# mburger-stsci/nexoclom

Measured on AMD Instinct MI355X. Metric: particle*steps/s, higher is better.
Workload: dtype f64

## Files before the change

### nexoclom_amd/build.py

```python
import os
import shutil
import subprocess
import sys

HERE = os.path.dirname(os.path.abspath(__file__))
SRC = os.path.join(HERE, 'csrc', 'nxc_api.hip')
DEPS = [os.path.join(HERE, 'csrc', f) for f in
        ('nxc_api.hip', 'nxc_kernels.hpp', 'nxc_device.hpp', 'nxc_math.hpp', 'nxc_log_table.hpp',
         'nxc_desc_check.hpp', 'nxc_source_limits.hpp')]
DEPS.append(os.path.join(os.path.dirname(HERE), 'include', 'nexoclom_hip.h'))
OUT = os.path.join(HERE, 'lib', 'libnexoclom_hip.so')
OUT_TWO_ROUNDINGS = os.path.join(HERE, 'lib', 'libnexoclom_hip_2r.so')

FLAGS = ['-O3', '--offload-arch=gfx950', '-ffp-contract=off', '-fno-fast-math',
         '-munsafe-fp-atomics', '-mllvm', '-disable-machine-licm', '-fPIC', '-shared',
         '-std=c++17', '-Wall', '-Wno-unused-function']
if os.environ.get('NXC_EXPERIMENT_KNOBS'):
    FLAGS.append('-DNXC_EXPERIMENT_KNOBS')
FLAGS += os.environ.get('NXC_EXTRA_FLAGS', '').split()


def hipcc():
    exe = shutil.which('hipcc') or '/opt/rocm/bin/hipcc'
    if not os.path.exists(exe):
        raise RuntimeError('hipcc not found; the HIP library cannot be built')
    return exe


def up_to_date(out=OUT):
    if not os.path.exists(out):
        return False
    t = os.path.getmtime(out)
# ... 32 lines not shown
```

### nexoclom_amd/csrc/nxc_api.hip

```cpp
#include <hip/hip_runtime.h>
#include <dlfcn.h>
#include <rccl/rccl.h>

#include <algorithm>
#include <atomic>
#include <cmath>
#include <cstddef>
#include <cstdio>
#include <cstdlib>
#include <cstring>
#include <ctime>
#include <limits>
#include <mutex>
#include <new>
#include <string>
#include <vector>

#include "../../include/nexoclom_hip.h"
#include "nxc_desc_check.hpp"
#include "nxc_kernels.hpp"
#include "nxc_log_table.hpp"

namespace {

// ... 70 lines not shown
    if (!g_rccl.lib) return fail(NXC_ERR_RCCL, std::string("dlopen(librccl): ") + dlerror());
#define SYM(field, name)                                                                     \
    g_rccl.field = reinterpret_cast<decltype(g_rccl.field)>(dlsym(g_rccl.lib, name));        \
    if (!g_rccl.field) return fail(NXC_ERR_RCCL, std::string("dlsym ") + name + " failed");
    SYM(GetUniqueId, "ncclGetUniqueId")
    SYM(CommInitRank, "ncclCommInitRank")
    SYM(AllReduce, "ncclAllReduce")
    SYM(CommDestroy, "ncclCommDestroy")
    SYM(CommAbort, "ncclCommAbort")
    SYM(CommGetAsyncError, "ncclCommGetAsyncError")
    SYM(GetErrorString, "ncclGetErrorString")
#undef SYM
    g_rccl.ok = true;
    return NXC_OK;
}

#define NCCLCHK(expr)                                                                        \
    do {                                                                                     \
        ncclResult_t r_ = (expr);                                                            \
        if (r_ != ncclSuccess)                                                               \
            return fail(NXC_ERR_RCCL, std::string(#expr) + ": " + g_rccl.GetErrorString(r_)); \
    } while (0)

struct PackedLut {
    LutDesc desc{};
    std::vector<unsigned char> bytes;
};
struct LosLutCache {
    int64_t n = 0;
    std::vector<double> v, g;
    PackedLut lut;
};

int lut_cell_host(double x, double xbase, double inv_w, int ncell)
{
    const double s = (x - xbase) * inv_w;
    long long c;
    if (!(s >= 0.0)) c = 0;
    else if (s >= 2147483647.0) c = 2147483647ll;
    else c = (long long)s;
    return (int)std::min<long long>(c, ncell + 1);
}

unsigned long long ordered_key(double v)
{
    unsigned long long b;
    std::memcpy(&b, &v, sizeof b);
    return (b >> 63) ? ~b : (b | 0x8000000000000000ull);
}
double from_ordered_key(unsigned long long k)
{
    const unsigned long long b = (k >> 63) ? (k & 0x7fffffffffffffffull) : ~k;
    double v;
    std::memcpy(&v, &b, sizeof v);
    return v;
}

int pack_lut(const double *xp, const double *fp, int64_t n, PackedLut &out, const char *what,
             int cells_per_node = 4)
{
    if (n < 2 || n > 65000 || !xp || !fp)
        return fail(NXC_ERR_ARG, std::string(what) + ": table needs 2..65000 points");
    for (int64_t j = 0; j + 1 < n; j++)
        if (!(xp[j + 1] > xp[j]))
            return fail(NXC_ERR_ARG, std::string(what) + ": abscissae must be strictly ascending");
    for (int64_t j = 0; j < n; j++)
        if (!std::isfinite(xp[j]) || !std::isfinite(fp[j]))
            return fail(NXC_ERR_ARG, std::string(what) + ": table values must be finite");
    int ncell = 64;
    while (ncell < cells_per_node * n && ncell < 16384) ncell <<= 1;
    const int64_t rows = n + 2;
    const size_t cell_bytes = ((size_t)(ncell + 2) * sizeof(unsigned short) + 31) & ~size_t(31);
    out.bytes.assign((size_t)rows * 32 + cell_bytes, 0);
    double *rec = reinterpret_cast<double *>(out.bytes.data());
    double *fs = rec + 2 * rows;
    rec[0] = -std::numeric_limits<double>::max(); rec[1] = xp[0];
    fs[0] = fp[0]; fs[1] = 0.0;
    for (int64_t j = 0; j < n; j++) {
        const bool last = j + 1 == n;
        rec[2 * (j + 1)] = xp[j];
        rec[2 * (j + 1) + 1] = last ? HUGE_VAL : xp[j + 1];
        fs[2 * (j + 1)] = fp[j];
        fs[2 * (j + 1) + 1] = last ? 0.0 : (fp[j + 1] - fp[j]) / (xp[j + 1] - xp[j]);
        if (!std::isfinite(fs[2 * (j + 1) + 1]))
            return fail(NXC_ERR_ARG, std::string(what) + ": table slopes must be finite");
    }
    rec[2 * (n + 1)] = HUGE_VAL; rec[2 * (n + 1) + 1] = HUGE_VAL;
    fs[2 * (n + 1)] = fp[n - 1]; fs[2 * (n + 1) + 1] = 0.0;
    const double x0 = xp[0], xl = xp[n - 1];
    const double inv_w = (double)ncell / (xl - x0);
    const double xbase = x0 - (xl - x0) / (double)ncell;
    if (!std::isfinite(inv_w) || !std::isfinite(xbase) || !(xbase < x0))
        return fail(NXC_ERR_ARG, std::string(what) + ": abscissa range cannot be indexed");
    unsigned short *cell = reinterpret_cast<unsigned short *>(rec + 4 * rows);
    cell[0] = 0;
    const unsigned long long k_lo = ordered_key(-std::numeric_limits<double>::max());
    const unsigned long long k_hi = ordered_key(std::numeric_limits<double>::max());
    for (int c = 1; c <= ncell + 1; c++) {
        if (lut_cell_host(from_ordered_key(k_hi), xbase, inv_w, ncell) < c)
            return fail(NXC_ERR_ARG, std::string(what) + ": cell index is not onto");
        unsigned long long lo = k_lo, hi = k_hi;
        while (hi - lo > 1) {
            const unsigned long long mid = lo + (hi - lo) / 2;
            if (lut_cell_host(from_ordered_key(mid), xbase, inv_w, ncell) >= c) hi = mid;
            else lo = mid;
        }
        const double first = from_ordered_key(hi);
        const int64_t j = std::upper_bound(xp, xp + n, first) - xp;
        cell[c] = (unsigned short)j;
    }
    out.desc.rec = 0;
    out.desc.fs = 16 * (int)rows;
    out.desc.cell = 32 * (int)rows;
    out.desc.top = ncell + 1;
    out.desc.last = (int)n + 1;
    out.desc.xbase = xbase;
    out.desc.inv_w = inv_w;
    return NXC_OK;
}

LutDesc placed_lut(LutDesc d, size_t base)
{
    d.rec += (int)base; d.fs += (int)base; d.cell += (int)base;
    return d;
}

double sqrt_threshold(double e)
{
    if (!(e > 0) || !std::isfinite(e)) return e;
    double x = e * e;
    if (!std::isfinite(x)) return HUGE_VAL;
    while (std::sqrt(x) > e) x = std::nextafter(x, 0.0);
    while (std::sqrt(std::nextafter(x, HUGE_VAL)) <= e) x = std::nextafter(x, HUGE_VAL);
    return x;
}

StepW make_stepw(double h)
{
    StepW w{};
    w.h = h;
    for (int n = 0; n < 6; n++)
        for (int i = 0; i <= n; i++) w.w[n * (n + 1) / 2 + i] = h * Tableau::A[n + 1][i];
    return w;
}

}

// ... 28 lines not shown
    const void *col0 = nullptr;
    int64_t stride = 0;
    template <typename T> const T *col(int c) const { return static_cast<const T *>(cols[c]); }
    template <typename I> const I *idx() const { return static_cast<const I *>(index); }
};

struct nxc_handle {
    int device = 0;
    int n_cu = 0;
    hipStream_t stream = nullptr;
    hipStream_t copy_stream = nullptr;
    hipStream_t stream2 = nullptr;
    unsigned long long *d_piece_hist = nullptr;
    hipEvent_t ev_piece[33] = {};
    hipEvent_t ev0 = nullptr, ev1 = nullptr;
    bool timed = false;
    char name[256] = {0};

    bool have_forces = false, have_image = false;
    ForceK F{};
    ImageK G{};
    PackedLut force_lut;
    std::vector<double> force_v, force_a;
    int force_cells_per_node = 16;
    int force_lut_cells = 0;
    std::vector<unsigned char> image_part;
    LdsHeader header{};
    LutDesc line_local[NXC_MAX_LINES]{};
    size_t line_start[NXC_MAX_LINES]{};
    int64_t xedges_local = 0, zedges_local = 0;
    unsigned char *d_blob = nullptr;
    size_t blob_cap = 0, force_bytes = 0, all_bytes = 0;
    unsigned char *d_blob_img = nullptr;
    size_t blob_img_cap = 0, img_bytes = 0;

    double *d_image = nullptr;
    size_t npix = 0;
    double *d_packets = nullptr;
    size_t packets_cap = 0;
    int64_t n_packets = 0;
    unsigned *d_order = nullptr;
    double *d_queue = nullptr;
    size_t queue_cap = 0;
    size_t order_cap = 0;
    bool have_order = false;
    int order_key = 0;
    int64_t first_id = 0;
    bool have_bounce = false;
// ... 250 lines not shown

std::mutex g_handles_lock;
std::vector<nxc_handle *> g_handles;

void flush_all_pools()
{
    std::lock_guard<std::mutex> g(g_handles_lock);
    for (nxc_handle *h : g_handles) pool_flush(h);
}

size_t pool_bytes(nxc_handle *h)
{
    std::lock_guard<std::mutex> g(h->pool.lock);
    return h->pool.bytes;
}

int upload_blob(nxc_handle *h)
{
    const size_t hb = NXC_HEADER_BYTES;
    const size_t ib = h->have_image ? h->image_part.size() : 0;
    const size_t limit = 160 * 1024 - 32 - (size_t)(BLOCK_PERSIST / 64) * NXC_WAVE_LDS_BYTES;
    const size_t limit_rows = 160 * 1024 - 32 - (size_t)(BLOCK_PERSIST / 64) * NXC_WAVE_LDS_BYTES_ROWS;
    size_t fb = h->have_forces ? h->force_lut.bytes.size() : 0;
    while (h->have_forces && (hb + fb + ib > limit || hb + fb > limit_rows) &&
           h->force_cells_per_node > 2) {
        h->force_cells_per_node /= 2;
        PackedLut lut;
        int rc2 = pack_lut(h->force_v.data(), h->force_a.data(), (int64_t)h->force_v.size(), lut,
                           "nxc_forces radiation table", h->force_cells_per_node);
        if (rc2) return rc2;
        h->force_lut = std::move(lut);
        h->force_lut_cells = h->force_cells_per_node;
        fb = h->force_lut.bytes.size();
    }
    h->force_bytes = hb + fb;
    h->all_bytes = hb + fb + ib;
    if (h->all_bytes > limit || h->force_bytes > limit_rows)
        return fail(NXC_ERR_ARG, "lookup tables exceed the 160 KiB LDS of a gfx950 CU");
    int rc = ensure(reinterpret_cast<void **>(&h->d_blob), &h->blob_cap, h->all_bytes);
    if (rc) return rc;
    h->F.tab = placed_lut(h->force_lut.desc, hb);
    if (h->have_image) {
        for (int l = 0; l < h->G.n_lines; l++) {
            h->G.line[l] = placed_lut(h->line_local[l], hb + fb + h->line_start[l]);
        }
        h->G.xedges_off = h->xedges_local + (int64_t)(hb + fb);
        h->G.zedges_off = h->zedges_local + (int64_t)(hb + fb);
    }
    h->header.G = h->G;
    HIPCHK(hipMemcpyAsync(h->d_blob, &h->header, sizeof(LdsHeader), hipMemcpyHostToDevice,
                          h->stream));
    if (fb) HIPCHK(hipMemcpyAsync(h->d_blob + hb, h->force_lut.bytes.data(), fb,
                                  hipMemcpyHostToDevice, h->stream));
    if (ib) HIPCHK(hipMemcpyAsync(h->d_blob + hb + fb, h->image_part.data(), ib,
                                  hipMemcpyHostToDevice, h->stream));
    HIPCHK(stream_sync(h));
    if (h->have_image) {
        LdsHeader hdr = h->header;
        for (int l = 0; l < h->G.n_lines; l++)
            hdr.G.line[l] = placed_lut(h->line_local[l], hb + h->line_start[l]);
        hdr.G.xedges_off = h->xedges_local + (int64_t)hb;
// ... 428 lines not shown
int los_tables(nxc_handle *h, const nxc_los_desc *d, LosK &K, std::vector<unsigned char> &blob)
{
    blob.assign((size_t)NXC_HEADER_BYTES, 0);
    std::memcpy(blob.data(), &h->header, sizeof(LdsHeader));
    K.sin_dphi = d->sin_dphi;
    K.sin_2dphi = d->sin_2dphi;
    K.cos_thr = d->cos_threshold;
    K.cos_thr2_lo = d->cos_threshold * d->cos_threshold * (1.0 - 1e-9);
    K.vrplanet = d->vrplanet;
    K.unit_cm2 = d->unit_cm * d->unit_cm;
    K.t0 = d->ladder[0];
    K.log1p_s_inv = 1.0 / std::log1p(d->sin_dphi);
    K.n_lines = d->n_lines;
    K.n_ladder = (int)d->n_ladder;
    K.tan_dphi = std::tan(d->dphi);
    for (int l = 0; l < d->n_lines; l++) {
        const size_t nb = (size_t)d->line_n[l] * sizeof(double);
        LosLutCache &c = h->los_lut[l];
        const bool same = c.n == d->line_n[l] && d->line_n[l] > 0 && c.v.size() * sizeof(double) == nb &&
                          std::memcmp(c.v.data(), d->line_v[l], nb) == 0 &&
                          std::memcmp(c.g.data(), d->line_g[l], nb) == 0;
        if (!same) {
            c.n = 0;
            int rc = pack_lut(d->line_v[l], d->line_g[l], d->line_n[l], c.lut, "g-value table");
            if (rc) return rc;
            c.v.assign(d->line_v[l], d->line_v[l] + d->line_n[l]);
            c.g.assign(d->line_g[l], d->line_g[l] + d->line_n[l]);
            c.n = d->line_n[l];
        }
        K.line[l] = placed_lut(c.lut.desc, blob.size());
        blob.insert(blob.end(), c.lut.bytes.begin(), c.lut.bytes.end());
    }
    return NXC_OK;
}

template <typename T, typename I>
int los_run(nxc_handle *h, const nxc_los_desc *d, int64_t S, const double *sc, int64_t P,
            const T *dx, const T *dy, const T *dz, const T *dvy, const T *dfrac, const I *d_index,
            int64_t index_shift, int64_t n_index, double *radiance, int64_t *npackets, uint8_t *included,
            int64_t used_cap, int64_t *used_pairs, int64_t *n_used)
{
    std::vector<unsigned char> blob;
    LosK K{};
    int rc = los_tables(h, d, K, blob);
    if (rc) return rc;
    K.index_shift = index_shift;
    K.cull = (d->dphi > 0 && d->dphi < 1.5 && std::isfinite(K.tan_dphi)) ? 1 : 0;
// ... 773 lines not shown
                          (unsigned long long)c.unfinished);
            return fail(NXC_ERR_INCOMPLETE, buf);
        }
    }
    return NXC_OK;
}

int nxc_set_forces(nxc_handle *h, const nxc_forces *f)
{
    return guarded([&]() -> int {
    if (!h || !f) return fail(NXC_ERR_ARG, "null argument");
    HIPCHK(hipSetDevice(h->device));
    PackedLut lut;
    const double zero_one[2] = {0.0, 1.0}, zeros[2] = {0.0, 0.0};
    int rc;
    const double *nv = f->radpres ? f->v_tab : zero_one, *na = f->radpres ? f->a_tab : zeros;
    const size_t nn = f->radpres ? (size_t)(f->n_tab > 0 ? f->n_tab : 0) : 2;
    if (f->radpres && (f->n_tab < 2 || !f->v_tab || !f->a_tab)) return fail(NXC_ERR_ARG, "radiation table missing");
    const bool same_table = h->have_forces && h->force_v.size() == nn && !h->force_lut.bytes.empty() &&
                            std::memcmp(h->force_v.data(), nv, nn * sizeof(double)) == 0 &&
                            std::memcmp(h->force_a.data(), na, nn * sizeof(double)) == 0;
    h->force_v.assign(nv, nv + nn);
    h->force_a.assign(na, na + nn);
    h->force_cells_per_node = 8;
#ifdef NXC_EXPERIMENT_KNOBS
    if (const char *e = std::getenv("NXC_FORCE_CELLS")) h->force_cells_per_node = std::max(2, std::atoi(e));
#endif
    if (!same_table || h->force_lut_cells != h->force_cells_per_node) {
        rc = pack_lut(h->force_v.data(), h->force_a.data(), (int64_t)h->force_v.size(), lut,
                      "nxc_forces radiation table", h->force_cells_per_node);
        if (rc) { h->have_forces = false; return rc; }
        h->force_lut = std::move(lut);
        h->force_lut_cells = h->force_cells_per_node;
    }
    h->F.GM = f->GM;
    h->F.vrplanet = f->vrplanet;
    h->F.photo = f->photo;
    h->F.inv_lifetime = f->lifetime > 0 ? 1.0 / f->lifetime : 0.0;
    h->F.grav = f->gravity ? 1 : 0;
    h->F.rad = f->radpres ? 1 : 0;
    h->F.loss = f->lifetime > 0 ? LOSS_LIFETIME : (f->has_photo ? LOSS_PHOTO : LOSS_NONE);
    h->have_forces = true;
    return upload_blob(h);
    });
}

int nxc_set_image(nxc_handle *h, const nxc_image_desc *d)
{
    return guarded([&]() -> int {
    if (!h || !d) return fail(NXC_ERR_ARG, "null argument");
    HIPCHK(hipSetDevice(h->device));
    if (d->nx < 1 || d->nz < 1 || d->nx > 32768 || d->nz > 32768 || !d->xedges || !d->zedges)
        return fail(NXC_ERR_ARG, "image dims/edges invalid");
    if (d->quantity != 0 && d->quantity != 1) return fail(NXC_ERR_ARG, "quantity must be 0 or 1");
    const int nl = d->quantity == 1 ? d->n_lines : 0;
    if (nl < 0 || nl > NXC_MAX_LINES) return fail(NXC_ERR_ARG, "n_lines out of range");
// ... 1 lines not shown
    if (!std::isfinite(d->vrplanet)) return fail(NXC_ERR_ARG, "vrplanet must be finite");
    for (int64_t k = 0; k < d->nx; k++)
        if (!(d->xedges[k + 1] > d->xedges[k])) return fail(NXC_ERR_ARG, "xedges not ascending");
    for (int64_t k = 0; k < d->nz; k++)
        if (!(d->zedges[k + 1] > d->zedges[k])) return fail(NXC_ERR_ARG, "zedges not ascending");

    std::vector<unsigned char> part;
    ImageK G{};
    std::memcpy(G.M, d->M, sizeof G.M);
    G.vrplanet = d->vrplanet;
    G.apix_cm2 = d->apix_cm2;
    G.quantity = d->quantity;
    G.n_lines = nl;
    G.downcast_f32 = d->downcast_f32 ? 1 : 0;
#ifdef NXC_EXPERIMENT_KNOBS
    if (const char *dbg = std::getenv("NXC_DEBUG_IMAGE")) G.dbg = std::atoi(dbg);
#endif
    G.nx = (int)d->nx;
    G.nz = (int)d->nz;
    G.x_is_x = (d->M[0] == 1.0 && d->M[1] == 0.0 && d->M[2] == 0.0 && d->M[3] == 0.0 &&
                d->M[6] == 0.0) ? 1 : 0;
    for (int l = 0; l < nl; l++) {
        PackedLut lut;
        int rc = pack_lut(d->line_v[l], d->line_g[l], d->line_n[l], lut, "g-value table");
        if (rc) return rc;
        h->line_local[l] = lut.desc;
        h->line_start[l] = part.size();
        part.insert(part.end(), lut.bytes.begin(), lut.bytes.end());
    }
    h->xedges_local = (int64_t)part.size();
    const unsigned char *xe = reinterpret_cast<const unsigned char *>(d->xedges);
    part.insert(part.end(), xe, xe + (d->nx + 1) * sizeof(double));
    h->zedges_local = (int64_t)part.size();
    const unsigned char *ze = reinterpret_cast<const unsigned char *>(d->zedges);
    part.insert(part.end(), ze, ze + (d->nz + 1) * sizeof(double));
    G.x_lo = d->xedges[0];
    G.x_inv_step = (double)d->nx / (d->xedges[d->nx] - d->xedges[0]);
    G.z_lo = d->zedges[0];
    G.z_inv_step = (double)d->nz / (d->zedges[d->nz] - d->zedges[0]);
    h->image_part = std::move(part);
    h->G = G;
    h->have_image = true;

    const size_t npix = (size_t)d->nx * (size_t)d->nz;
    if (npix != h->npix) {
        if (h->d_image) HIPCHK(hipFree(h->d_image));
        h->d_image = nullptr; h->npix = 0;
// ... 1643 lines not shown
    const std::vector<u128> maps = pcg_tables(((u128)inc[0] << 64) | inc[1], n);
    const size_t map_bytes = maps.size() * sizeof(u128), out_bytes = (size_t)nvec * count * 8;
    int rc = scratch_for(h, map_bytes + out_bytes);
    if (rc) return rc;
    unsigned char *base = reinterpret_cast<unsigned char *>(h->d_scratch);
    HIPCHK(hipMemcpyAsync(base, maps.data(), map_bytes, hipMemcpyHostToDevice, h->stream));
    PcgK P{};
    P.state = ((u128)state[0] << 64) | state[1];
    P.row0 = row0;
    P.maps = reinterpret_cast<const nxc_u128 *>(base);
    hipLaunchKernelGGL(k_pcg_uniforms, dim3(flat_grid(h, count, NXC_BLOCK)), dim3(NXC_BLOCK), 0,
                       h->stream, P, (int)nvec, count, reinterpret_cast<double *>(base + map_bytes));
    HIPCHK(hipGetLastError());
    HIPCHK(hipMemcpyAsync(out, base + map_bytes, out_bytes, hipMemcpyDeviceToHost, h->stream));
    HIPCHK(stream_sync(h));
    return NXC_OK;
    });
}

int nxc_math_batch(nxc_handle *h, int which, int64_t n, const double *in, const double *in2,
                   double *out)
{
    return guarded([&]() -> int {
    if (!h || n < 0 || (n && (!in || !out)) || which < 0 || which > 4 || (which == 4 && !in2))
        return fail(NXC_ERR_ARG, "bad arguments");
    HIPCHK(hipSetDevice(h->device));
    if (n == 0) return NXC_OK;
    const size_t col = (size_t)n * sizeof(double);
    int rc = scratch_for(h, 3 * col);
    if (rc) return rc;
    double *d = h->d_scratch;
    HIPCHK(hipMemcpyAsync(d, in, col, hipMemcpyHostToDevice, h->stream));
    if (in2) HIPCHK(hipMemcpyAsync(d + n, in2, col, hipMemcpyHostToDevice, h->stream));
    if (!h->d_blob && (rc = upload_blob(h))) return rc;
    hipLaunchKernelGGL(k_math, dim3(flat_grid(h, n, 256)), dim3(256), NXC_HEADER_BYTES, h->stream,
                       h->d_blob, which, n, d, d + n, d + 2 * n);
    HIPCHK(hipGetLastError());
    HIPCHK(hipMemcpyAsync(out, d + 2 * n, col, hipMemcpyDeviceToHost, h->stream));
    HIPCHK(stream_sync(h));
    return NXC_OK;
    });
}

}
```

### nexoclom_amd/csrc/nxc_device.hpp

```cpp
#pragma once
#include <hip/hip_runtime.h>
#include <stdint.h>
#include "nxc_math.hpp"

struct LutDesc {
    int rec, fs, cell;
    int top;
    int last;
    int pad_;
    double xbase;
    double inv_w;
};
typedef LutDesc LutView;

extern __shared__ __align__(32) unsigned char nxc_lds[];

#define NXC_LDS_AS __attribute__((address_space(3)))
#define NXC_GLOBAL_AS __attribute__((address_space(1)))
typedef double nxc_v2d __attribute__((ext_vector_type(2)));

NXC_DEV double lds_f64(int byte_off)
{
    return *(const NXC_LDS_AS double *)(unsigned)byte_off;
}
NXC_DEV int lds_u16(int byte_off)
{
    return *(const NXC_LDS_AS unsigned short *)(unsigned)byte_off;
}

NXC_DEV double2 lds_f64x2(int byte_off)
{
    const nxc_v2d v = *(const NXC_LDS_AS nxc_v2d *)(unsigned)byte_off;
    return make_double2(v.x, v.y);
}

NXC_DEV const LutView &lut_view(const LutDesc &d) { return d; }

NXC_DEV int lut_cell(const LutView &t, double x)
{
    const double s = (x - t.xbase) * t.inv_w;
    unsigned c;
    asm("v_cvt_u32_f64 %0, %1" : "=v"(c) : "v"(s));
    const unsigned top = (unsigned)t.top;
    return (int)(c > top ? top : c);
}

struct LutProbe {
    double x;
    int r;
    double2 a0, a1, b0, b1;
};

NXC_DEV void lut_probe_cell(const LutView &t, double x, LutProbe &p)
{
    p.x = x;
    p.r = lds_u16(t.cell + 2 * lut_cell(t, x));
}

NXC_DEV void lut_probe_rows(const LutView &t, LutProbe &p)
{
    const int ra = t.rec + 16 * p.r, rb = t.fs + 16 * p.r;
    p.a0 = lds_f64x2(ra); p.a1 = lds_f64x2(ra + 16);
    p.b0 = lds_f64x2(rb); p.b1 = lds_f64x2(rb + 16);
}

NXC_DEV LutProbe lut_probe(const LutView &t, double x)
{
    LutProbe p;
    lut_probe_cell(t, x, p);
    lut_probe_rows(t, p);
    return p;
}

NXC_DEV double lut_finish(const LutView &t, const LutProbe &p)
{
    const double x = p.x;
    const bool in0 = x < p.a0.y, in1 = x < p.a1.y;
    double xp = in0 ? p.a0.x : p.a1.x;
    double fp = in0 ? p.b0.x : p.b1.x;
    double sl = in0 ? p.b0.y : p.b1.y;
    if (__builtin_expect(!(in0 || in1), 0)) {
        int r = p.r + 1;
        while (r < t.last && x >= lds_f64(t.rec + 16 * r + 8)) ++r;
        const double2 aw = lds_f64x2(t.rec + 16 * r), bw = lds_f64x2(t.fs + 16 * r);
        xp = aw.x; fp = bw.x; sl = bw.y;
    }
    return sl * (x - xp) + fp;
}

NXC_DEV double lut_interp(const LutView &t, double x) { return lut_finish(t, lut_probe(t, x)); }

enum : int { LOSS_NONE = 0, LOSS_LIFETIME = 1, LOSS_PHOTO = 2 };

struct ForceK {
    double GM, vrplanet, photo, inv_lifetime;
    int grav, rad, loss, pad_;
    LutDesc tab;
};

NXC_DEV bool sunlit(double x, double y, double z)
{
    double s = x * x + z * z;
    return (s > 0x1.0000000000001p+0) || (y < 0.0);
}

template <bool FULL>
NXC_DEV void state_eval(const ForceK &F, const LutView &T, double x, double y, double z, double vy,
                        double &ax, double &ay, double &az, double &ion)
{
    const bool lit = sunlit(x, y, z);
// ... 633 lines not shown
NXC_DEV bool image_weight(const ImageK &G, const ImageRegs &R, double radvel, double fw,
                          double &w_out)
{
    double w = fw;
    if (R.quantity != 0) {
        double gg = 0.0;
        if (R.n_lines == 2) {
            const LutView v0 = lut_view(G.line[0]), v1 = lut_view(G.line[1]);
            LutProbe p0, p1;
            lut_probe_cell(v0, radvel, p0); lut_probe_cell(v1, radvel, p1);
            lut_probe_rows(v0, p0); lut_probe_rows(v1, p1);
            const double g0 = lut_finish(v0, p0);
            gg = g0 + lut_finish(v1, p1);
        } else {
            gg = R.n_lines > 0 ? lut_interp(lut_view(G.line[0]), radvel) : 0.0;
#pragma unroll
            for (int l = 1; l < 4; l++)
                if (l < R.n_lines) gg += lut_interp(lut_view(G.line[l]), radvel);
        }
        w = nxc_div_const(fw * gg, 1e6, lds_header().Wt.rs_1e6);
    }
    w = nxc_div_const(w, G.apix_cm2, lds_header().Wt.rs_apix);
    w_out = w;
    return (__builtin_fabs(w) <= 1.7976931348623157e308) && radvel == radvel;
}

NXC_DEV void image_sample(const ImageK &G, const ImageRegs &R, bool has, double x, double y,
                          double z, double vy, double frac, double *__restrict__ acc2,
                          unsigned long long &binned, unsigned long long &nonfinite)
{
    int pix = -1;
    double radvel = 0.0, fw = 0.0, w = 0.0;
    if (has) pix = image_locate(G, R, x, y, z, vy, frac, radvel, fw, nonfinite);
    bool ok = pix >= 0;
    if (ok && !image_weight(G, R, radvel, fw, w)) { nonfinite++; ok = false; }
    binned += ok;
    image_add_pairs(ok, pix, w, acc2);
}

constexpr int NXC_IMGQ_SLOTS = 128;
constexpr int NXC_IMGQ_BYTES = NXC_IMGQ_SLOTS * (8 + 8 + 4);

struct ImageQueue {
    int head = 0, tail = 0;

    NXC_DEV void push(bool has, int pix, double radvel, double fw, int qoff)
    {
// ... 63 lines not shown
```

### nexoclom_amd/csrc/nxc_kernels.hpp

```cpp
#pragma once
#include "nxc_device.hpp"
#include "nxc_source_limits.hpp"

struct DevCounters {
    unsigned long long particle_steps, samples, samples_binned, nonfinite, bad_step, neg_frac,
        unfinished, queue_head;
    unsigned long long wave_trips;
#ifdef NXC_STAMPS
    unsigned long long stamp[8];
#endif
};

#ifdef NXC_STAMPS
NXC_DEV unsigned long long nxc_stamp()
{
    unsigned long long t;
    __builtin_amdgcn_sched_barrier(0);
    asm volatile("s_memtime %0\n\ts_waitcnt lgkmcnt(0)" : "=s"(t) : : "memory");
    __builtin_amdgcn_sched_barrier(0);
    return t;
}
#define NXC_STAMP(k) do { const unsigned long long t_ = nxc_stamp(); seg[k] += t_ - t_prev; t_prev = t_; } while (0)
#else
#define NXC_STAMP(k) do { } while (0)
// ... 1072 lines not shown
#pragma unroll
    for (int j = 0; j < 8; j++) sink += a[j];
    const unsigned long long t1 = __builtin_amdgcn_s_memtime(), r1 = __builtin_amdgcn_s_memrealtime();
    if ((threadIdx.x & 63) == 0) {
        const size_t w = ((size_t)blockIdx.x * blockDim.x + threadIdx.x) >> 6;
        out[3 * w] = t1 - t0;
        out[3 * w + 1] = r1 - r0;
        out[3 * w + 2] = (unsigned long long)__double_as_longlong(sink);
    }
}

__global__ void __launch_bounds__(64)
k_stall(unsigned long long ticks, unsigned long long *__restrict__ out)
{
    const unsigned long long t0 = __builtin_amdgcn_s_memrealtime();
    unsigned long long now = t0;
    while (now - t0 < ticks) {
        __builtin_amdgcn_s_sleep(127);
        now = __builtin_amdgcn_s_memrealtime();
    }
    if (threadIdx.x == 0 && out) *out = now - t0;
}

__global__ void k_math(const unsigned char *__restrict__ blob, int which, int64_t n,
                       const double *__restrict__ in, const double *__restrict__ in2,
                       double *__restrict__ out)
{
    stage_tables(blob, NXC_HEADER_BYTES);
    for (int64_t i = (int64_t)blockIdx.x * blockDim.x + threadIdx.x; i < n;
         i += (int64_t)gridDim.x * blockDim.x) {
        const double v = in[i];
        double r;
        switch (which) {
        case 0: r = nxc_exp(v); break;
        case 1: r = nxc_log(v); break;
        case 2: r = nxc_cube(v); break;
        case 3: r = nxc_sqrt(v); break;
        default: r = nxc_div(v, in2[i]); break;
        }
        out[i] = r;
    }
}

struct LosK {
    double sin_dphi, sin_2dphi, cos_thr, cos_thr2_lo, vrplanet, unit_cm2;
    double log1p_s_inv, t0;
    double tan_dphi;
    int cull, tile_cap;
    int n_lines, n_ladder;
    int64_t index_shift;
    int64_t row_base;
    int64_t tile_off;
    LutDesc line[4];
};

constexpr int NXC_LOS_TILE = 512;
constexpr int NXC_LOS_SP = 7;
#ifndef NXC_LOS_BLOCK_N
#define NXC_LOS_BLOCK_N 8
#endif
constexpr int NXC_LOS_BLOCK = NXC_LOS_BLOCK_N;

NXC_DEV bool los_pair_maybe(const LosK &K, const double *__restrict__ sp, double px, double py, double pz)
{
    const double rx = px - sp[0], ry = py - sp[1], rz = pz - sp[2];
    const double q = (rx * sp[3] + ry * sp[4]) + rz * sp[5];
    if (!(q > 0.0) || !(q < sp[6])) return false;
    const double d2 = (rx * rx + ry * ry) + rz * rz;
    return q * q >= K.cos_thr2_lo * d2;
}

NXC_DEV double los_wtemp(const LosK &K, double vy_p, double frac_p, double dist, double rs_1e6,
                         unsigned long long &my_nonfinite)
{
    const double radvel = vy_p + K.vrplanet;
    double gg = K.n_lines > 0 ? lut_interp(lut_view(K.line[0]), radvel) : 0.0;
#pragma unroll
    for (int l = 1; l < 4; l++)
        if (l < K.n_lines) gg += lut_interp(lut_view(K.line[l]), radvel);
    const double weight = nxc_div_const(frac_p * gg, 1e6, rs_1e6);
    if (!(__builtin_fabs(weight) <= 1.7976931348623157e308) || radvel != radvel) my_nonfinite++;
    const double ds = dist * K.sin_dphi;
    const double apix = (3.141592653589793 * (ds * ds)) * K.unit_cm2;
    return nxc_div(weight, apix);
}

NXC_DEV void los_pair(const LosK &K, const double *__restrict__ sp, int64_t spectrum, int64_t p,
                      double px, double py, double pz, double vy_p, double frac_p, long long idx_p,
                      const double *ladder, double *radiance, unsigned long long *npackets,
                      unsigned char *__restrict__ included, long long used_cap,
                      long long *__restrict__ used_pairs, unsigned long long *__restrict__ n_used,
                      double rs_1e6, unsigned long long &my_pairs, unsigned long long &my_nonfinite)
{
    const double xs = sp[0], ys = sp[1], zs = sp[2], bx = sp[3], by = sp[4], bz = sp[5];
    const double rx = px - xs, ry = py - ys, rz = pz - zs;
    const double q = (rx * bx + ry * by) + rz * bz;
    if (!(q > 0.0) || !(q < sp[6])) return;
    const double d2 = (rx * rx + ry * ry) + rz * rz;
    if (!(q * q >= K.cos_thr2_lo * d2)) return;
#if defined(NXC_LOS_EXPERIMENT) && NXC_LOS_EXPERIMENT >= 1
    my_pairs++;
    return;
#endif
    const double dist = nxc_sqrt(d2);
// ... 1409 lines not shown
```

### nexoclom_amd/hip_api.py

```python
import ctypes as C
import os
import threading
import weakref

import numpy as np

_HERE = os.path.dirname(os.path.abspath(__file__))
LIB_PATH = os.environ.get('NEXOCLOM_HIP_LIB') or os.path.join(_HERE, 'lib', 'libnexoclom_hip.so')
_dp = C.POINTER(C.c_double)
NXC_MAX_LINES = 4
NXC_RUN_IMAGE = 1
NXC_UNIQUE_ID_BYTES = 128

EXPORTS = ('nxc_abi_version', 'nxc_device_count', 'nxc_last_error_string', 'nxc_create',
           'nxc_destroy', 'nxc_device_name', 'nxc_synchronize', 'nxc_set_forces',
           'nxc_set_image', 'nxc_state', 'nxc_rk5_step', 'nxc_packets_upload', 'nxc_image_clear',
           'nxc_image_download', 'nxc_counters_get', 'nxc_last_kernel_ms', 'nxc_integrate_const',
           'nxc_integrate_const_async', 'nxc_integrate_var', 'nxc_image_accumulate',
           'nxc_image_accumulate_f32',
           'nxc_comm_unique_id', 'nxc_comm_init', 'nxc_comm_destroy', 'nxc_image_allreduce',
           'nxc_allreduce_max_f64', 'nxc_barrier', 'nxc_math_batch', 'nxc_los_accumulate',
           'nxc_los_accumulate_f32', 'nxc_packets_sample',
           'nxc_set_bounce', 'nxc_set_first_index', 'nxc_set_bodies',
           'nxc_integrate_const_rows', 'nxc_rows_fetch', 'nxc_rows_fetch_f32', 'nxc_device_bus_id',
# ... 884 lines not shown

    def comm_test_stall(self, seconds):
        self._check(self.lib.nxc_comm_test_stall(self._h, C.c_double(seconds)))

    def stream_copy_gbs(self, nbytes=1 << 31, reps=5):
        gbs = C.c_double(0)
        self._check(self.lib.nxc_stream_copy_gbs(self._h, C.c_int64(nbytes), C.c_int(reps),
                                                 C.byref(gbs)))
        return float(gbs.value)

    def shader_clock_mhz(self):
        mhz = C.c_double(0)
        self._check(self.lib.nxc_shader_clock_mhz(self._h, C.byref(mhz)))
        return float(mhz.value)

    def pcg64_uniforms(self, seed, n, row0, count, nvec):
        state, inc = pcg64_words(seed)
        out = np.empty((nvec, count))
        self._check(self.lib.nxc_pcg64_uniforms(self._h, state, inc, C.c_int64(n), C.c_int64(row0),
                                                C.c_int64(count), C.c_int32(nvec), _p(out)))
        return out

    def math(self, which, x, y=None):
        code = {'exp': 0, 'log': 1, 'cube': 2, 'sqrt': 3, 'div': 4}[which]
        x = _f64(x)
        out = np.empty_like(x)
        y2 = _f64(y) if y is not None else None
        self._check(self.lib.nxc_math_batch(self._h, C.c_int(code), C.c_int64(len(x)), _p(x),
                                            _p(y2) if y2 is not None else None, _p(out)))
        return out
```

Baseline: 33.67 billion.

## Redesign LDS lookup table with per-cell split keys and separate slope array

Reworks the packed interpolation table: each cell now holds up to three split abscissae plus a base row index in one 32-byte entry, so a lookup does branch-free comparisons and then reads one (x,f) pair and one slope, instead of reading two rows of record and slope data and choosing between them. Rows shrink from 32 to 24 bytes, and the default density becomes two nodes per cell, which changes how much LDS the tables take. Cells with more than three nodes, and the edge cells, fall back to a linear walk. Also adds a host reference interpolator, a lookup mode in the math test kernel, and a stricter nonfinite check on radvel.

```diff
diff --git a/nexoclom_amd/build.py b/nexoclom_amd/build.py
--- a/nexoclom_amd/build.py
+++ b/nexoclom_amd/build.py
@@ -7,7 +7,7 @@
 SRC = os.path.join(HERE, 'csrc', 'nxc_api.hip')
 DEPS = [os.path.join(HERE, 'csrc', f) for f in
         ('nxc_api.hip', 'nxc_kernels.hpp', 'nxc_device.hpp', 'nxc_math.hpp', 'nxc_log_table.hpp',
-         'nxc_desc_check.hpp', 'nxc_source_limits.hpp')]
+         'nxc_desc_check.hpp', 'nxc_source_limits.hpp', 'nxc_lut_pack.hpp')]
 DEPS.append(os.path.join(os.path.dirname(HERE), 'include', 'nexoclom_hip.h'))
 OUT = os.path.join(HERE, 'lib', 'libnexoclom_hip.so')
 OUT_TWO_ROUNDINGS = os.path.join(HERE, 'lib', 'libnexoclom_hip_2r.so')
diff --git a/nexoclom_amd/csrc/nxc_api.hip b/nexoclom_amd/csrc/nxc_api.hip
--- a/nexoclom_amd/csrc/nxc_api.hip
+++ b/nexoclom_amd/csrc/nxc_api.hip
@@ -116,107 +116,17 @@
             return fail(NXC_ERR_RCCL, std::string(#expr) + ": " + g_rccl.GetErrorString(r_)); \
     } while (0)
 
-struct PackedLut {
-    LutDesc desc{};
-    std::vector<unsigned char> bytes;
-};
 struct LosLutCache {
     int64_t n = 0;
     std::vector<double> v, g;
     PackedLut lut;
 };
 
-int lut_cell_host(double x, double xbase, double inv_w, int ncell)
-{
-    const double s = (x - xbase) * inv_w;
-    long long c;
-    if (!(s >= 0.0)) c = 0;
-    else if (s >= 2147483647.0) c = 2147483647ll;
-    else c = (long long)s;
-    return (int)std::min<long long>(c, ncell + 1);
-}
-
-unsigned long long ordered_key(double v)
-{
-    unsigned long long b;
-    std::memcpy(&b, &v, sizeof b);
-    return (b >> 63) ? ~b : (b | 0x8000000000000000ull);
-}
-double from_ordered_key(unsigned long long k)
-{
-    const unsigned long long b = (k >> 63) ? (k & 0x7fffffffffffffffull) : ~k;
-    double v;
-    std::memcpy(&v, &b, sizeof v);
-    return v;
-}
-
-int pack_lut(const double *xp, const double *fp, int64_t n, PackedLut &out, const char *what,
-             int cells_per_node = 4)
-{
-    if (n < 2 || n > 65000 || !xp || !fp)
-        return fail(NXC_ERR_ARG, std::string(what) + ": table needs 2..65000 points");
-    for (int64_t j = 0; j + 1 < n; j++)
-        if (!(xp[j + 1] > xp[j]))
-            return fail(NXC_ERR_ARG, std::string(what) + ": abscissae must be strictly ascending");
-    for (int64_t j = 0; j < n; j++)
-        if (!std::isfinite(xp[j]) || !std::isfinite(fp[j]))
-            return fail(NXC_ERR_ARG, std::string(what) + ": table values must be finite");
-    int ncell = 64;
-    while (ncell < cells_per_node * n && ncell < 16384) ncell <<= 1;
-    const int64_t rows = n + 2;
-    const size_t cell_bytes = ((size_t)(ncell + 2) * sizeof(unsigned short) + 31) & ~size_t(31);
-    out.bytes.assign((size_t)rows * 32 + cell_bytes, 0);
-    double *rec = reinterpret_cast<double *>(out.bytes.data());
-    double *fs = rec + 2 * rows;
-    rec[0] = -std::numeric_limits<double>::max(); rec[1] = xp[0];
-    fs[0] = fp[0]; fs[1] = 0.0;
-    for (int64_t j = 0; j < n; j++) {
-        const bool last = j + 1 == n;
-        rec[2 * (j + 1)] = xp[j];
-        rec[2 * (j + 1) + 1] = last ? HUGE_VAL : xp[j + 1];
-        fs[2 * (j + 1)] = fp[j];
-        fs[2 * (j + 1) + 1] = last ? 0.0 : (fp[j + 1] - fp[j]) / (xp[j + 1] - xp[j]);
-        if (!std::isfinite(fs[2 * (j + 1) + 1]))
-            return fail(NXC_ERR_ARG, std::string(what) + ": table slopes must be finite");
-    }
-    rec[2 * (n + 1)] = HUGE_VAL; rec[2 * (n + 1) + 1] = HUGE_VAL;
-    fs[2 * (n + 1)] = fp[n - 1]; fs[2 * (n + 1) + 1] = 0.0;
-    const double x0 = xp[0], xl = xp[n - 1];
-    const double inv_w = (double)ncell / (xl - x0);
-    const double xbase = x0 - (xl - x0) / (double)ncell;
-    if (!std::isfinite(inv_w) || !std::isfinite(xbase) || !(xbase < x0))
-        return fail(NXC_ERR_ARG, std::string(what) + ": abscissa range cannot be indexed");
-    unsigned short *cell = reinterpret_cast<unsigned short *>(rec + 4 * rows);
-    cell[0] = 0;
-    const unsigned long long k_lo = ordered_key(-std::numeric_limits<double>::max());
-    const unsigned long long k_hi = ordered_key(std::numeric_limits<double>::max());
-    for (int c = 1; c <= ncell + 1; c++) {
-        if (lut_cell_host(from_ordered_key(k_hi), xbase, inv_w, ncell) < c)
-            return fail(NXC_ERR_ARG, std::string(what) + ": cell index is not onto");
-        unsigned long long lo = k_lo, hi = k_hi;
-        while (hi - lo > 1) {
-            const unsigned long long mid = lo + (hi - lo) / 2;
-            if (lut_cell_host(from_ordered_key(mid), xbase, inv_w, ncell) >= c) hi = mid;
-            else lo = mid;
-        }
-        const double first = from_ordered_key(hi);
-        const int64_t j = std::upper_bound(xp, xp + n, first) - xp;
-        cell[c] = (unsigned short)j;
-    }
-    out.desc.rec = 0;
-    out.desc.fs = 16 * (int)rows;
-    out.desc.cell = 32 * (int)rows;
-    out.desc.top = ncell + 1;
-    out.desc.last = (int)n + 1;
-    out.desc.xbase = xbase;
-    out.desc.inv_w = inv_w;
-    return NXC_OK;
-}
-
-LutDesc placed_lut(LutDesc d, size_t base)
-{
-    d.rec += (int)base; d.fs += (int)base; d.cell += (int)base;
-    return d;
+int pack_lut_or_fail(const double *xp, const double *fp, int64_t n, PackedLut &out, const char *what,
+                     int nodes_per_cell = NXC_LUT_NODES_PER_CELL)
+{
+    const std::string why = pack_lut(xp, fp, n, out, what, nodes_per_cell);
+    return why.empty() ? NXC_OK : fail(NXC_ERR_ARG, why);
 }
 
 double sqrt_threshold(double e)
@@ -291,8 +201,8 @@
     ImageK G{};
     PackedLut force_lut;
     std::vector<double> force_v, force_a;
-    int force_cells_per_node = 16;
-    int force_lut_cells = 0;
+    int force_nodes_per_cell = NXC_LUT_NODES_PER_CELL;
+    int force_lut_nodes = 0;
     std::vector<unsigned char> image_part;
     LdsHeader header{};
     LutDesc line_local[NXC_MAX_LINES]{};
@@ -589,21 +499,21 @@
     const size_t limit = 160 * 1024 - 32 - (size_t)(BLOCK_PERSIST / 64) * NXC_WAVE_LDS_BYTES;
     const size_t limit_rows = 160 * 1024 - 32 - (size_t)(BLOCK_PERSIST / 64) * NXC_WAVE_LDS_BYTES_ROWS;
     size_t fb = h->have_forces ? h->force_lut.bytes.size() : 0;
-    while (h->have_forces && (hb + fb + ib > limit || hb + fb > limit_rows) &&
-           h->force_cells_per_node > 2) {
-        h->force_cells_per_node /= 2;
+    while (h->have_forces && !lut_budget_refusal(hb, fb, ib, limit, limit_rows).empty() &&
+           h->force_nodes_per_cell < 16) {
+        h->force_nodes_per_cell *= 2;
         PackedLut lut;
-        int rc2 = pack_lut(h->force_v.data(), h->force_a.data(), (int64_t)h->force_v.size(), lut,
-                           "nxc_forces radiation table", h->force_cells_per_node);
+        int rc2 = pack_lut_or_fail(h->force_v.data(), h->force_a.data(), (int64_t)h->force_v.size(),
+                                   lut, "nxc_forces radiation table", h->force_nodes_per_cell);
         if (rc2) return rc2;
         h->force_lut = std::move(lut);
-        h->force_lut_cells = h->force_cells_per_node;
+        h->force_lut_nodes = h->force_nodes_per_cell;
         fb = h->force_lut.bytes.size();
     }
     h->force_bytes = hb + fb;
     h->all_bytes = hb + fb + ib;
-    if (h->all_bytes > limit || h->force_bytes > limit_rows)
-        return fail(NXC_ERR_ARG, "lookup tables exceed the 160 KiB LDS of a gfx950 CU");
+    const std::string why = lut_budget_refusal(hb, fb, ib, limit, limit_rows);
+    if (!why.empty()) return fail(NXC_ERR_ARG, why);
     int rc = ensure(reinterpret_cast<void **>(&h->d_blob), &h->blob_cap, h->all_bytes);
     if (rc) return rc;
     h->F.tab = placed_lut(h->force_lut.desc, hb);
@@ -1078,7 +988,7 @@
                           std::memcmp(c.g.data(), d->line_g[l], nb) == 0;
         if (!same) {
             c.n = 0;
-            int rc = pack_lut(d->line_v[l], d->line_g[l], d->line_n[l], c.lut, "g-value table");
+            int rc = pack_lut_or_fail(d->line_v[l], d->line_g[l], d->line_n[l], c.lut, "g-value table");
             if (rc) return rc;
             c.v.assign(d->line_v[l], d->line_v[l] + d->line_n[l]);
             c.g.assign(d->line_g[l], d->line_g[l] + d->line_n[l]);
@@ -1898,16 +1808,16 @@
                             std::memcmp(h->force_a.data(), na, nn * sizeof(double)) == 0;
     h->force_v.assign(nv, nv + nn);
     h->force_a.assign(na, na + nn);
-    h->force_cells_per_node = 8;
+    h->force_nodes_per_cell = NXC_LUT_NODES_PER_CELL;
 #ifdef NXC_EXPERIMENT_KNOBS
-    if (const char *e = std::getenv("NXC_FORCE_CELLS")) h->force_cells_per_node = std::max(2, std::atoi(e));
+    if (const char *e = std::getenv("NXC_FORCE_NODES_PER_CELL")) h->force_nodes_per_cell = std::max(1, std::atoi(e));
 #endif
-    if (!same_table || h->force_lut_cells != h->force_cells_per_node) {
-        rc = pack_lut(h->force_v.data(), h->force_a.data(), (int64_t)h->force_v.size(), lut,
-                      "nxc_forces radiation table", h->force_cells_per_node);
+    if (!same_table || h->force_lut_nodes != h->force_nodes_per_cell) {
+        rc = pack_lut_or_fail(h->force_v.data(), h->force_a.data(), (int64_t)h->force_v.size(), lut,
+                              "nxc_forces radiation table", h->force_nodes_per_cell);
         if (rc) { h->have_forces = false; return rc; }
         h->force_lut = std::move(lut);
-        h->force_lut_cells = h->force_cells_per_node;
+        h->force_lut_nodes = h->force_nodes_per_cell;
     }
     h->F.GM = f->GM;
     h->F.vrplanet = f->vrplanet;
@@ -1955,7 +1865,7 @@
                 d->M[6] == 0.0) ? 1 : 0;
     for (int l = 0; l < nl; l++) {
         PackedLut lut;
-        int rc = pack_lut(d->line_v[l], d->line_g[l], d->line_n[l], lut, "g-value table");
+        int rc = pack_lut_or_fail(d->line_v[l], d->line_g[l], d->line_n[l], lut, "g-value table");
         if (rc) return rc;
         h->line_local[l] = lut.desc;
         h->line_start[l] = part.size();
@@ -3645,8 +3555,9 @@
                    double *out)
 {
     return guarded([&]() -> int {
-    if (!h || n < 0 || (n && (!in || !out)) || which < 0 || which > 4 || (which == 4 && !in2))
+    if (!h || n < 0 || (n && (!in || !out)) || which < 0 || which > 5 || (which == 4 && !in2))
         return fail(NXC_ERR_ARG, "bad arguments");
+    if (which == 5 && !h->have_forces) return fail(NXC_ERR_STATE, "nxc_math_batch: the lookup needs nxc_set_forces");
     HIPCHK(hipSetDevice(h->device));
     if (n == 0) return NXC_OK;
     const size_t col = (size_t)n * sizeof(double);
@@ -3656,8 +3567,10 @@
     HIPCHK(hipMemcpyAsync(d, in, col, hipMemcpyHostToDevice, h->stream));
     if (in2) HIPCHK(hipMemcpyAsync(d + n, in2, col, hipMemcpyHostToDevice, h->stream));
     if (!h->d_blob && (rc = upload_blob(h))) return rc;
-    hipLaunchKernelGGL(k_math, dim3(flat_grid(h, n, 256)), dim3(256), NXC_HEADER_BYTES, h->stream,
-                       h->d_blob, which, n, d, d + n, d + 2 * n);
+    const size_t staged = which == 5 ? h->force_bytes : (size_t)NXC_HEADER_BYTES;
+    if ((rc = prep_kernel(k_math, staged))) return rc;
+    hipLaunchKernelGGL(k_math, dim3(flat_grid(h, n, 256)), dim3(256), staged, h->stream, h->d_blob,
+                       (int64_t)staged, h->F.tab, which, n, d, d + n, d + 2 * n);
     HIPCHK(hipGetLastError());
     HIPCHK(hipMemcpyAsync(out, d + 2 * n, col, hipMemcpyDeviceToHost, h->stream));
     HIPCHK(stream_sync(h));
diff --git a/nexoclom_amd/csrc/nxc_device.hpp b/nexoclom_amd/csrc/nxc_device.hpp
--- a/nexoclom_amd/csrc/nxc_device.hpp
+++ b/nexoclom_amd/csrc/nxc_device.hpp
@@ -3,14 +3,7 @@
 #include <stdint.h>
 #include "nxc_math.hpp"
 
-struct LutDesc {
-    int rec, fs, cell;
-    int top;
-    int last;
-    int pad_;
-    double xbase;
-    double inv_w;
-};
+#include "nxc_lut_pack.hpp"
 typedef LutDesc LutView;
 
 extern __shared__ __align__(32) unsigned char nxc_lds[];
@@ -23,11 +16,6 @@
 {
     return *(const NXC_LDS_AS double *)(unsigned)byte_off;
 }
-NXC_DEV int lds_u16(int byte_off)
-{
-    return *(const NXC_LDS_AS unsigned short *)(unsigned)byte_off;
-}
-
 NXC_DEV double2 lds_f64x2(int byte_off)
 {
     const nxc_v2d v = *(const NXC_LDS_AS nxc_v2d *)(unsigned)byte_off;
@@ -47,21 +35,31 @@
 
 struct LutProbe {
     double x;
-    int r;
-    double2 a0, a1, b0, b1;
+    double2 c0, c1;
+    double2 xf;
+    double sl;
 };
 
 NXC_DEV void lut_probe_cell(const LutView &t, double x, LutProbe &p)
 {
     p.x = x;
-    p.r = lds_u16(t.cell + 2 * lut_cell(t, x));
+    const int ca = t.cell + NXC_LUT_CELL_BYTES * lut_cell(t, x);
+    p.c0 = lds_f64x2(ca); p.c1 = lds_f64x2(ca + 16);
 }
 
 NXC_DEV void lut_probe_rows(const LutView &t, LutProbe &p)
 {
-    const int ra = t.rec + 16 * p.r, rb = t.fs + 16 * p.r;
-    p.a0 = lds_f64x2(ra); p.a1 = lds_f64x2(ra + 16);
-    p.b0 = lds_f64x2(rb); p.b1 = lds_f64x2(rb + 16);
+    const double x = p.x;
+    int r = __double2loint(p.c1.y);
+    r += (int)(x >= p.c0.x);
+    r += (int)(x >= p.c0.y);
+    r += (int)(x >= p.c1.x);
+    if (__builtin_expect(__double2hiint(p.c1.y) != 0, 0)) {
+        while (r < t.last && x >= lds_f64(t.xf + 16 * r + 16)) ++r;
+        if (__builtin_isinf(x)) p.x = lds_f64(t.xf + 16 * r);
+    }
+    p.xf = lds_f64x2(t.xf + 16 * r);
+    p.sl = lds_f64(t.sl + 8 * r);
 }
 
 NXC_DEV LutProbe lut_probe(const LutView &t, double x)
@@ -72,20 +70,9 @@
     return p;
 }
 
-NXC_DEV double lut_finish(const LutView &t, const LutProbe &p)
-{
-    const double x = p.x;
-    const bool in0 = x < p.a0.y, in1 = x < p.a1.y;
-    double xp = in0 ? p.a0.x : p.a1.x;
-    double fp = in0 ? p.b0.x : p.b1.x;
-    double sl = in0 ? p.b0.y : p.b1.y;
-    if (__builtin_expect(!(in0 || in1), 0)) {
-        int r = p.r + 1;
-        while (r < t.last && x >= lds_f64(t.rec + 16 * r + 8)) ++r;
-        const double2 aw = lds_f64x2(t.rec + 16 * r), bw = lds_f64x2(t.fs + 16 * r);
-        xp = aw.x; fp = bw.x; sl = bw.y;
-    }
-    return sl * (x - xp) + fp;
+NXC_DEV double lut_finish(const LutView &, const LutProbe &p)
+{
+    return p.sl * (p.x - p.xf.x) + p.xf.y;
 }
 
 NXC_DEV double lut_interp(const LutView &t, double x) { return lut_finish(t, lut_probe(t, x)); }
@@ -765,7 +752,8 @@
     }
     w = nxc_div_const(w, G.apix_cm2, lds_header().Wt.rs_apix);
     w_out = w;
-    return (__builtin_fabs(w) <= 1.7976931348623157e308) && radvel == radvel;
+    return (__builtin_fabs(w) <= 1.7976931348623157e308) &&
+           (__builtin_fabs(radvel) <= 1.7976931348623157e308);
 }
 
 NXC_DEV void image_sample(const ImageK &G, const ImageRegs &R, bool has, double x, double y,
diff --git a/nexoclom_amd/csrc/nxc_kernels.hpp b/nexoclom_amd/csrc/nxc_kernels.hpp
--- a/nexoclom_amd/csrc/nxc_kernels.hpp
+++ b/nexoclom_amd/csrc/nxc_kernels.hpp
@@ -1118,11 +1118,11 @@
     if (threadIdx.x == 0 && out) *out = now - t0;
 }
 
-__global__ void k_math(const unsigned char *__restrict__ blob, int which, int64_t n,
-                       const double *__restrict__ in, const double *__restrict__ in2,
-                       double *__restrict__ out)
-{
-    stage_tables(blob, NXC_HEADER_BYTES);
+__global__ void k_math(const unsigned char *__restrict__ blob, int64_t stage_bytes, LutDesc tab,
+                       int which, int64_t n, const double *__restrict__ in,
+                       const double *__restrict__ in2, double *__restrict__ out)
+{
+    stage_tables(blob, stage_bytes);
     for (int64_t i = (int64_t)blockIdx.x * blockDim.x + threadIdx.x; i < n;
          i += (int64_t)gridDim.x * blockDim.x) {
         const double v = in[i];
@@ -1132,6 +1132,7 @@
         case 1: r = nxc_log(v); break;
         case 2: r = nxc_cube(v); break;
         case 3: r = nxc_sqrt(v); break;
+        case 5: r = lut_interp(lut_view(tab), v); break;
         default: r = nxc_div(v, in2[i]); break;
         }
         out[i] = r;
@@ -1175,7 +1176,8 @@
     for (int l = 1; l < 4; l++)
         if (l < K.n_lines) gg += lut_interp(lut_view(K.line[l]), radvel);
     const double weight = nxc_div_const(frac_p * gg, 1e6, rs_1e6);
-    if (!(__builtin_fabs(weight) <= 1.7976931348623157e308) || radvel != radvel) my_nonfinite++;
+    if (!(__builtin_fabs(weight) <= 1.7976931348623157e308) ||
+        !(__builtin_fabs(radvel) <= 1.7976931348623157e308)) my_nonfinite++;
     const double ds = dist * K.sin_dphi;
     const double apix = (3.141592653589793 * (ds * ds)) * K.unit_cm2;
     return nxc_div(weight, apix);
diff --git a/nexoclom_amd/csrc/nxc_lut_pack.hpp b/nexoclom_amd/csrc/nxc_lut_pack.hpp
--- /dev/null
+++ b/nexoclom_amd/csrc/nxc_lut_pack.hpp
@@ -0,0 +1,188 @@
+#pragma once
+
+#include <algorithm>
+#include <cmath>
+#include <cstddef>
+#include <cstdint>
+#include <cstring>
+#include <limits>
+#include <string>
+#include <vector>
+
+struct LutDesc {
+    int xf, sl, cell;
+    int top;
+    int last;
+    int pad_;
+    double xbase;
+    double inv_w;
+};
+
+constexpr int NXC_LUT_SPLITS = 3;
+constexpr int NXC_LUT_CELL_BYTES = 32;
+constexpr int NXC_LUT_NODES_PER_CELL = 2;
+
+struct PackedLut {
+    LutDesc desc{};
+    std::vector<unsigned char> bytes;
+};
+
+inline int lut_cell_host(double x, double xbase, double inv_w, int ncell)
+{
+    const double s = (x - xbase) * inv_w;
+    long long c;
+    if (!(s >= 0.0)) c = 0;
+    else if (s >= 2147483647.0) c = 2147483647ll;
+    else c = (long long)s;
+    return (int)std::min<long long>(c, ncell + 1);
+}
+
+inline unsigned long long ordered_key(double v)
+{
+    unsigned long long b;
+    std::memcpy(&b, &v, sizeof b);
+    return (b >> 63) ? ~b : (b | 0x8000000000000000ull);
+}
+inline double from_ordered_key(unsigned long long k)
+{
+    const unsigned long long b = (k >> 63) ? (k & 0x7fffffffffffffffull) : ~k;
+    double v;
+    std::memcpy(&v, &b, sizeof v);
+    return v;
+}
+
+inline size_t lut_bytes(int64_t n, int ncell)
+{
+    const size_t rows = (size_t)n + 1;
+    const size_t row_bytes = (rows * 24 + 31) & ~size_t(31);
+    return row_bytes + (size_t)(ncell + 2) * NXC_LUT_CELL_BYTES;
+}
+
+inline int lut_ncell(int64_t n, int nodes_per_cell)
+{
+    int ncell = 64;
+    while ((int64_t)ncell * nodes_per_cell < n && ncell < 16384) ncell <<= 1;
+    return ncell;
+}
+
+inline bool lut_cell_starts(double xbase, double inv_w, int ncell, std::vector<double> &first)
+{
+    const unsigned long long k_lo = ordered_key(-std::numeric_limits<double>::max());
+    const unsigned long long k_hi = ordered_key(std::numeric_limits<double>::max());
+    if (lut_cell_host(from_ordered_key(k_hi), xbase, inv_w, ncell) < ncell + 1) return false;
+    first.assign((size_t)ncell + 3, 0.0);
+    first[0] = -HUGE_VAL;
+    first[(size_t)ncell + 2] = HUGE_VAL;
+    for (int c = 1; c <= ncell + 1; c++) {
+        unsigned long long lo = k_lo, hi = k_hi;
+        while (hi - lo > 1) {
+            const unsigned long long mid = lo + (hi - lo) / 2;
+            if (lut_cell_host(from_ordered_key(mid), xbase, inv_w, ncell) >= c) hi = mid;
+            else lo = mid;
+        }
+        first[c] = from_ordered_key(hi);
+        if (lut_cell_host(first[c], xbase, inv_w, ncell) != c) return false;
+    }
+    return true;
+}
+
+inline std::string pack_lut(const double *xp, const double *fp, int64_t n, PackedLut &out,
+                            const char *what, int nodes_per_cell = NXC_LUT_NODES_PER_CELL)
+{
+    if (n < 2 || n > 65000 || !xp || !fp)
+        return std::string(what) + ": table needs 2..65000 points";
+    if (nodes_per_cell < 1) return std::string(what) + ": nodes per cell must be positive";
+    for (int64_t j = 0; j + 1 < n; j++)
+        if (!(xp[j + 1] > xp[j]))
+            return std::string(what) + ": abscissae must be strictly ascending";
+    for (int64_t j = 0; j < n; j++)
+        if (!std::isfinite(xp[j]) || !std::isfinite(fp[j]))
+            return std::string(what) + ": table values must be finite";
+    const int ncell = lut_ncell(n, nodes_per_cell);
+    const int64_t rows = n + 1;
+    const size_t sl_off = (size_t)rows * 16;
+    const size_t cell_off = ((size_t)rows * 24 + 31) & ~size_t(31);
+    out.bytes.assign(lut_bytes(n, ncell), 0);
+    double *xf = reinterpret_cast<double *>(out.bytes.data());
+    double *sl = reinterpret_cast<double *>(out.bytes.data() + sl_off);
+    xf[0] = -std::numeric_limits<double>::max(); xf[1] = fp[0];
+    sl[0] = 0.0;
+    for (int64_t j = 0; j < n; j++) {
+        xf[2 * (j + 1)] = xp[j];
+        xf[2 * (j + 1) + 1] = fp[j];
+        sl[j + 1] = j + 1 == n ? 0.0 : (fp[j + 1] - fp[j]) / (xp[j + 1] - xp[j]);
+        if (!std::isfinite(sl[j + 1]))
+            return std::string(what) + ": table slopes must be finite";
+    }
+    const double x0 = xp[0], xl = xp[n - 1];
+    const double inv_w = (double)ncell / (xl - x0);
+    const double xbase = x0 - (xl - x0) / (double)ncell;
+    if (!std::isfinite(inv_w) || !std::isfinite(xbase) || !(xbase < x0))
+        return std::string(what) + ": abscissa range cannot be indexed";
+    std::vector<double> first;
+    if (!lut_cell_starts(xbase, inv_w, ncell, first))
+        return std::string(what) + ": cell index is not onto";
+    unsigned char *cells = out.bytes.data() + cell_off;
+    for (int c = 0; c <= ncell + 1; c++) {
+        const int64_t row = std::upper_bound(xp, xp + n, first[c]) - xp;
+        const int64_t inside = (std::lower_bound(xp, xp + n, first[(size_t)c + 1]) - xp) - row;
+        double e[4];
+        for (int k = 0; k < NXC_LUT_SPLITS; k++)
+            e[k] = k < inside ? xp[row + k] : std::numeric_limits<double>::quiet_NaN();
+        const bool rare = inside > NXC_LUT_SPLITS || c == 0 || c == ncell + 1;
+        const unsigned long long word = (unsigned long long)row | ((unsigned long long)rare << 32);
+        std::memcpy(&e[3], &word, sizeof word);
+        std::memcpy(cells + (size_t)c * NXC_LUT_CELL_BYTES, e, sizeof e);
+    }
+    out.desc.xf = 0;
+    out.desc.sl = (int)sl_off;
+    out.desc.cell = (int)cell_off;
+    out.desc.top = ncell + 1;
+    out.desc.last = (int)n;
+    out.desc.pad_ = 0;
+    out.desc.xbase = xbase;
+    out.desc.inv_w = inv_w;
+    return "";
+}
+
+inline std::string lut_budget_refusal(size_t header_bytes, size_t force_bytes, size_t image_bytes,
+                                      size_t limit, size_t limit_rows)
+{
+    const size_t all = header_bytes + force_bytes + image_bytes;
+    if (all <= limit && header_bytes + force_bytes <= limit_rows) return "";
+    return "lookup tables exceed the 160 KiB LDS of a gfx950 CU: " + std::to_string(all) +
+           " bytes staged (" + std::to_string(force_bytes) + " radiation table, " +
+           std::to_string(image_bytes) + " image tables and edges), " + std::to_string(limit) +
+           " fit beside the per-wave blocks (" + std::to_string(limit_rows) +
+           " when rows are written)";
+}
+
+inline LutDesc placed_lut(LutDesc d, size_t base)
+{
+    d.xf += (int)base; d.sl += (int)base; d.cell += (int)base;
+    return d;
+}
+
+inline double lut_interp_host(const PackedLut &t, double x, int *cell_out = nullptr,
+                              int *splits = nullptr, int *walked = nullptr)
+{
+    const unsigned char *b = t.bytes.data();
+    const int c = lut_cell_host(x, t.desc.xbase, t.desc.inv_w, t.desc.top - 1);
+    double e[4];
+    std::memcpy(e, b + t.desc.cell + (size_t)c * NXC_LUT_CELL_BYTES, sizeof e);
+    unsigned long long word;
+    std::memcpy(&word, &e[3], sizeof word);
+    const int hit = (int)(x >= e[0]) + (int)(x >= e[1]) + (int)(x >= e[2]);
+    int r = (int)(word & 0xffffffffull) + hit, w = -1;
+    const double *xf = reinterpret_cast<const double *>(b + t.desc.xf);
+    const double *sl = reinterpret_cast<const double *>(b + t.desc.sl);
+    if (word >> 32) {
+        w = 0;
+        while (r < t.desc.last && x >= xf[2 * (r + 1)]) { ++r; ++w; }
+        if (std::isinf(x)) x = xf[2 * r];
+    }
+    if (cell_out) *cell_out = c;
+    if (splits) *splits = hit;
+    if (walked) *walked = w;
+    return sl[r] * (x - xf[2 * r]) + xf[2 * r + 1];
+}
diff --git a/nexoclom_amd/hip_api.py b/nexoclom_amd/hip_api.py
--- a/nexoclom_amd/hip_api.py
+++ b/nexoclom_amd/hip_api.py
@@ -930,7 +930,7 @@
         return out
 
     def math(self, which, x, y=None):
-        code = {'exp': 0, 'log': 1, 'cube': 2, 'sqrt': 3, 'div': 4}[which]
+        code = {'exp': 0, 'log': 1, 'cube': 2, 'sqrt': 3, 'div': 4, 'lookup': 5}[which]
         x = _f64(x)
         out = np.empty_like(x)
         y2 = _f64(y) if y is not None else None
```

After: 34.37 billion, median of 6. 2.1% higher.
